# asharakeh/pod_compare

Measured on AMD Instinct MI355X. Metric: images/sec (BayesOD+MC-dropout, 1280x720), higher is better.
Workload: dtype f32 (convolutions: every fp32 product from 2-way f16 splits of the power-of-two-scaled fp32 operands, 3 partial products, fp32 accumulate; closer to fp64 than the fp32 MFMA: profiles/r05_f16_split_numerics.txt)

## Files before the change

pod_compare_amd/csrc/k12_wino_conv_split.hip:

```cpp
#include "pod_wino.h"

namespace pod {

typedef uint32_t vu32x4 __attribute__((ext_vector_type(4)));
constexpr int WINO_US_BYTES = 24 * 2 * 2 * 64 * 16;
constexpr int WINO_U_TOP = 14, WINO_V_TOP = 9;
constexpr int WINO_WAIT_VM24 = 0x4078;
constexpr int WINO_TAIL_NO_LOAD = 1, WINO_TAIL_NO_PARK = 2, WINO_TAIL_LAST = 4;

__global__ void __launch_bounds__(256) k_wino_filter_amax(const float* __restrict__ w, float* __restrict__ amax, int32_t K, int32_t C, int32_t Kpad) {
    const int64_t t = (int64_t)blockIdx.x * blockDim.x + threadIdx.x;
    float m = 0.0f;
    if (t < (int64_t)Kpad * C) {
        float u[4][6];
        wino_filter_values(w, (int)(t / C), (int)(t % C), K, C, u);
#pragma unroll
        for (int i = 0; i < 24; ++i) m = fmaxf(m, fabsf(u[i / 6][i % 6]));
    }
    wino_publish_amax1(amax, m);
}
__global__ void __launch_bounds__(256) k_wino_filter_split(const float* __restrict__ w, uint16_t* __restrict__ Us, const float* __restrict__ amax,
                                                           int32_t K, int32_t C, int32_t Kpad) {
    const int64_t t = (int64_t)blockIdx.x * blockDim.x + threadIdx.x;
    if (t >= (int64_t)Kpad * C) return;
    const int k = (int)(t / C), c = (int)(t % C);
    float u[4][6];
    wino_filter_values(w, k, c, K, C, u);
    const float sc = wino_pow2_scale(*amax, WINO_U_TOP);
    const int nchunk = C / 16, ks = k >> 6, kb = (k >> 5) & 1, j32 = k & 31, ch = c >> 4, hh = (c >> 3) & 1, e = c & 7;
    uint16_t* dst = Us + (((int64_t)ks * nchunk + ch) * (int64_t)WINO_US_BYTES) / 2 + (hh * 32 + j32) * 8 + e;
#pragma unroll
    for (int a = 0; a < 4; ++a)
#pragma unroll
        for (int p = 0; p < 6; ++p) {
            const float x = u[a][p] * sc;
            const _Float16 h0 = (_Float16)x;
            const _Float16 h1 = (_Float16)(x - (float)h0);
            uint16_t* d = dst + (((a * 6 + p) * 2 + kb) * 2) * 512;
            d[0] = __builtin_bit_cast(uint16_t, h0);
            d[512] = __builtin_bit_cast(uint16_t, h1);
        }
}

__global__ void __launch_bounds__(256, 1) k_wino_conv3x3_split(const WinoParams P) {
    extern __shared__ __attribute__((aligned(16))) float lds[];
    const int tid = threadIdx.x, lane = tid & 63, wave = tid >> 6;
    int ks, tb;
    wino_schedule(P.KS, P.n_blocks, ks, tb);
    if (tb >= P.n_blocks) return;
    uint32_t need[2] = {~0u, ~0u};
    if (P.live) {
        if (tb >= P.live[0]) return;
        const int32_t* const ent = P.live + POD_SPARSE_LIVE_HEAD + (int64_t)POD_SPARSE_LIVE_STRIDE * tb;
        tb = ent[0];
        need[0] = (uint32_t)ent[1 + (tid >> 5)];
        need[1] = (uint32_t)ent[9 + (tid >> 5 < 3 ? tid >> 5 : 2)];
    }
    WINO_STAMP(0);
    WINO_STAMP_WALL(12);
    uint32_t slot_e[12];
    int mini_pidx[3], dmini[3], doff[12];
    WINO_FILL_SLOTS(slot_e, mini_pidx, tid);
    const int nchunk_all = P.C >> 4;
    const int nchunk = P.c_split ? P.c_split : nchunk_all;
    const int chunk0 = (int)blockIdx.y * nchunk;
    const int i32 = lane & 31, h = lane >> 5;
    const int a = __builtin_amdgcn_readfirstlane(wave);
    const int set = (tb >= P.sets.first[1] ? 1 : 0) + (tb >= P.sets.first[2] ? 1 : 0) + (tb >= P.sets.first[3] ? 1 : 0);
    const float* const set_U = P.sets.U[set];
    const float* const set_in = P.sets.in[set];
    float* const set_out = P.sets.out[set];
    const float* const set_bias = P.sets.bias[set];
    const float in_amax_slot = wino_load_amax(P.sets.in_amax[set]);
    const float u_amax = *reinterpret_cast<const float*>(reinterpret_cast<const char*>(set_U) + (int64_t)P.KS * (P.C >> 4) * WINO_US_BYTES);
    float* const set_out_amax = P.sets.out_amax[set];
    const uint64_t set_offset = P.sets.offset[set];
    const int set_replicas = P.sets.replicas[set], set_k_planes = P.sets.k_planes[set];
    const auto u_rsrc = __builtin_amdgcn_make_buffer_rsrc(const_cast<char*>(reinterpret_cast<const char*>(set_U) + ((int64_t)ks * nchunk_all + chunk0) * WINO_US_BYTES), 0,
                                                          nchunk * WINO_US_BYTES, 0x00020000);
    const int u_off = (a * 6 * 4 * 64 + h * 32 + i32) * 16;
    constexpr int WINO_U_LEAD = 3;
    vu32x4 uP[6][4];
    auto filter_piece = [&](int q16, int p, vu32x4(&u)[4], int i) {
        u[i] = __builtin_bit_cast(vu32x4, __builtin_amdgcn_raw_buffer_load_b128(u_rsrc, u_off, q16 * WINO_US_BYTES + (p * 4 + i) * 1024, 0));
    };
#pragma unroll
    for (int pp = 0; pp < WINO_U_LEAD; ++pp)
#pragma unroll
        for (int i = 0; i < 4; ++i) filter_piece(0, pp, uP[pp], i);
    const WinoBlock B = wino_block(P.blocks[tb]);
    int row0, row1;
    float sgn;
    wino_rows(a, row0, row1, sgn);
    const int ty = i32 >> 2, tx = i32 & 3;
    const uint32_t lds_base = (uint32_t)(uintptr_t)(__attribute__((address_space(3))) float*)lds;
    uint32_t areg[2][2][2][2];
    uint32_t amini[2];
#pragma unroll
    for (int rs = 0; rs < 2; ++rs) {
        const int py = 2 * ty + (rs ? row1 : row0);
        const int p0 = 2 * (((py & 3) + 4 * (py >> 3)) * 18 + 4 * tx) + ((py >> 2) & 1);
#pragma unroll
        for (int cl = 0; cl < 2; ++cl) {
            const int rot = ((tx + cl) & 3) + 4 * ((py >> 1) & 1);
#pragma unroll
            for (int c16 = 0; c16 < 2; ++c16)
#pragma unroll
                for (int hf = 0; hf < 2; ++hf) areg[rs][cl][c16][hf] = lds_base + p0 * 128 + ((4 * c16 + 2 * h + hf + rot) & 7) * 16;
        }
    }
#pragma unroll
    for (int rs = 0; rs < 2; ++rs) amini[rs] = lds_base + 2 * WINO_SB_FLOATS * 4 + h * 12288 + ((2 * ty + (rs ? row1 : row0)) * 21 + tx) * 32;
    const auto r_rsrc = __builtin_amdgcn_make_buffer_rsrc(const_cast<float*>(set_in + B.base_px * P.in_stride + chunk0 * 16), 0,
                                                          B.n_img * B.HWi * P.in_stride * 4 - chunk0 * 64, 0x00020000);
    int* const pix_tab = wino_pixel_table(lds);
    WINO_FILL_PIXEL_TABLE(pix_tab, B, need, tid);
    wino_mini_offsets(&P, pix_tab, mini_pidx, dmini, lane);
    auto main_offsets = [&]() {
#pragma unroll
        for (int i = 0; i < 12; ++i) doff[i] = pix_tab[slot_e[i] & 0xFFFF];
#pragma unroll
        for (int i = 0; i < 12; ++i) doff[i] = wino_byte_offset(&P, doff[i], 4 * (((lane & 7) - (int)(slot_e[i] >> 16)) & 7));
    };

    f32x4 stg[6];
    const uint32_t stg_addr = lds_base + a * 12288 + lane * 16;
    auto stage_load = [&](int k, int sc, int i) {
        stg[k] = __builtin_bit_cast(f32x4, __builtin_amdgcn_raw_buffer_load_b128(r_rsrc, doff[i], sc * 128, 0));
    };
    auto stage_write = [&](int par, int k, int i) {
        *reinterpret_cast<__attribute__((address_space(3))) f32x4*>((uintptr_t)(stg_addr + par * (WINO_SB_FLOATS * 4) + i * 1024)) = stg[k];
    };

    f32x16 acc[12];
    f32x4 x[12];
    vu32x4 Vb[6][2];
    float tN[6][4], vN[2][6][4];
    if (POD_WINO_ELIM) {
#pragma unroll
    for (int i = 0; i < 12; ++i) Vb[i / 2][i % 2] = vu32x4{0x3c003c00u + i, 0x3c003c00u, 0x3c003c00u, 0x3c003c00u + lane};
#pragma unroll
    for (int i = 0; i < 12; ++i) x[i] = f32x4{1e-3f, 2e-3f, 3e-3f, 4e-3f} * (float)(lane + i);
#pragma unroll
    for (int i = 0; i < 48; ++i) vN[i / 24][(i / 4) % 6][i % 4] = x[i / 4][i % 4];
#pragma unroll
    for (int i = 0; i < 24; ++i) tN[i / 4][i % 4] = x[i / 4][i % 4];
    }
#define WINO_READ(par, c16, hf, i)                                                                                                  \
    asm volatile("ds_read_b128 %0, %1 offset:%2" : "=v"(x[i]) : "v"(areg[(i) / 6][((i) % 6) >> 2][c16][hf]), "i"((par) * WINO_SB_FLOATS * 4 + ((i) % 6) * 256))
#define WINO_READ_MINI(hf, i)                                                                                                        \
    asm volatile("ds_read_b128 %0, %1 offset:%2" : "=v"(x[i]) : "v"(amini[(i) / 6]), "i"((hf) * 16 + ((((i) % 6) & 3) * 5 + (((i) % 6) >> 2)) * 32))
#define WINO_READ12(M, ...)                                                                                                          \
    M(__VA_ARGS__, 0); M(__VA_ARGS__, 1); M(__VA_ARGS__, 2); M(__VA_ARGS__, 3); M(__VA_ARGS__, 4); M(__VA_ARGS__, 5);                \
    M(__VA_ARGS__, 6); M(__VA_ARGS__, 7); M(__VA_ARGS__, 8); M(__VA_ARGS__, 9); M(__VA_ARGS__, 10); M(__VA_ARGS__, 11)
#define WINO_READS_LANDED()                                                                                                           \
    asm volatile("s_waitcnt lgkmcnt(0)" : "+v"(x[0]), "+v"(x[1]), "+v"(x[2]), "+v"(x[3]), "+v"(x[4]), "+v"(x[5]), "+v"(x[6]), "+v"(x[7]), \
                 "+v"(x[8]), "+v"(x[9]), "+v"(x[10]), "+v"(x[11]))
    auto rows_combine = [&](int c0, int c1) __attribute__((always_inline)) {
#pragma unroll
        for (int c = c0; c < c1; ++c) {
#pragma unroll
            for (int e = 0; e < 4; ++e) tN[c][e] = __builtin_fmaf(sgn, x[6 + c][e], x[c][e]);
        }
    };
    float w0s[4], w1s[4], evs[4], ods[4], fs[4], gs[4];
    auto columns_level1 = [&](int e) __attribute__((always_inline)) {
        w0s[e] = __builtin_fmaf(-5.0f, tN[2][e], tN[4][e]);
        w1s[e] = __builtin_fmaf(-5.0f, tN[3][e], tN[5][e]);
        evs[e] = __builtin_fmaf(-4.0f, tN[2][e], tN[4][e]);
        ods[e] = __builtin_fmaf(-4.0f, tN[1][e], tN[3][e]);
        fs[e] = tN[4][e] - tN[2][e];
        gs[e] = tN[3][e] - tN[1][e];
    };
    auto columns_level2 = [&](int hf, int e) __attribute__((always_inline)) {
        vN[hf][0][e] = __builtin_fmaf(4.0f, tN[0][e], w0s[e]);
        vN[hf][5][e] = __builtin_fmaf(4.0f, tN[1][e], w1s[e]);
        vN[hf][1][e] = evs[e] + ods[e];
        vN[hf][2][e] = evs[e] - ods[e];
        vN[hf][3][e] = __builtin_fmaf(2.0f, gs[e], fs[e]);
        vN[hf][4][e] = __builtin_fmaf(-2.0f, gs[e], fs[e]);
    };
    const float sv = __builtin_bit_cast(float, __builtin_amdgcn_readfirstlane(__builtin_bit_cast(int, wino_pow2_scale(wino_reduce_amax(in_amax_slot), WINO_V_TOP))));
    auto split_convert = [&](int p, int term) __attribute__((always_inline)) {
        vu32x4 w;
#pragma unroll
        for (int i = 0; i < 4; ++i) {
            w[i] = term == 0 ? wino_f16_pair_scaled(vN[i >> 1][p][2 * (i & 1)], vN[i >> 1][p][2 * (i & 1) + 1], sv)
                             : wino_f16_pair(vN[i >> 1][p][2 * (i & 1)], vN[i >> 1][p][2 * (i & 1) + 1]);
        }
        Vb[p][term] = w;
    };
    auto split_residual = [&](int p, int i0, int i1) __attribute__((always_inline)) {
#pragma unroll
        for (int i = i0; i < i1; ++i) {
            float& lo = vN[i >> 1][p][2 * (i & 1)];
            float& hi = vN[i >> 1][p][2 * (i & 1) + 1];
            wino_f16_residual_scaled(Vb[p][0][i], lo, hi, sv);
        }
    };
    auto split_position = [&](int p) __attribute__((always_inline)) {
        split_convert(p, 0); split_residual(p, 0, 4); split_convert(p, 1);
    };
    auto make_v = [&](int hf) __attribute__((always_inline)) {
        if (POD_WINO_ELIM & 8) return;
        rows_combine(0, 6);
#pragma unroll
        for (int e = 0; e < 4; ++e) columns_level1(e);
#pragma unroll
        for (int e = 0; e < 4; ++e) columns_level2(hf, e);
    };
    auto split_all = [&]() __attribute__((always_inline)) {
        if (POD_WINO_ELIM & 8) return;
#pragma unroll
        for (int p = 0; p < 6; ++p) split_position(p);
    };

    constexpr int N_UNITS = 58, N_SLOTS = 36;
    auto unit = [&](auto U, auto npar_t, auto n16_t, auto hasA_t) __attribute__((always_inline)) {
        constexpr int u = decltype(U)::value, npar = decltype(npar_t)::value, n16 = decltype(n16_t)::value;
        if constexpr (POD_WINO_ELIM & 8) { if constexpr (u >= 3 && !(u >= 13 && u < 16)) return; }
        if constexpr (u < 3) {
            if constexpr (!(POD_WINO_ELIM & 1)) { WINO_READ(npar, n16, 0, 4 * u); WINO_READ(npar, n16, 0, 4 * u + 1); WINO_READ(npar, n16, 0, 4 * u + 2); WINO_READ(npar, n16, 0, 4 * u + 3); }
        } else if constexpr (u < 7) {
            if constexpr (decltype(hasA_t)::value) {
                constexpr int k = u - 3;
                if constexpr (k == 0) split_convert(5, 0);
                else if constexpr (k == 1) split_residual(5, 0, 2);
                else if constexpr (k == 2) split_residual(5, 2, 4);
                else split_convert(5, 1);
            }
        } else if constexpr (u < 13) {
            if constexpr (u == 7) WINO_READS_LANDED();
            rows_combine(u - 7, u - 6);
        } else if constexpr (u < 16) {
            if constexpr (!(POD_WINO_ELIM & 1)) { WINO_READ(npar, n16, 1, 4 * (u - 13)); WINO_READ(npar, n16, 1, 4 * (u - 13) + 1); WINO_READ(npar, n16, 1, 4 * (u - 13) + 2); WINO_READ(npar, n16, 1, 4 * (u - 13) + 3); }
        } else if constexpr (u < 24) {
            constexpr int k = u - 16;
            if constexpr (k < 4) columns_level1(k);
            else columns_level2(0, k - 4);
        } else if constexpr (u < 30) {
            if constexpr (u == 24) WINO_READS_LANDED();
            rows_combine(u - 24, u - 23);
        } else if constexpr (u < 38) {
            constexpr int k = u - 30;
            if constexpr (k < 4) columns_level1(k);
            else columns_level2(1, k - 4);
        } else {
            constexpr int p = (u - 38) / 4, k = (u - 38) % 4;
            if constexpr (k == 0) split_convert(p, 0);
            else if constexpr (k == 1) split_residual(p, 0, 2);
            else if constexpr (k == 2) split_residual(p, 2, 4);
            else split_convert(p, 1);
        }
    };
    const int last = nchunk - 1, last_s = last >> 1;
    const int sc1 = last_s < 1 ? last_s : 1;
#pragma unroll
    for (int r = 0; r < 3; ++r) wino_mini_piece(r_rsrc, lds, a, 0, r, dmini[r]);
#pragma unroll
    for (int r = 0; r < 3; ++r) wino_mini_piece(r_rsrc, lds, a, 1, r, dmini[r]);
    WINO_STAMP(9);
    main_offsets();
    WINO_STAMP(10);
#pragma unroll
    for (int i = 0; i < 12; ++i) wino_patch_piece(r_rsrc, lds, a, 0, i, doff[i]);
#pragma unroll
    for (int i = 0; i < 6; ++i) wino_patch_piece(r_rsrc, lds + WINO_SB_FLOATS, a, sc1, i, doff[i]);
#pragma unroll
    for (int i = 0; i < 6; ++i) stage_load(i, sc1, 6 + i);
    WINO_STAMP(11);
    __builtin_amdgcn_s_waitcnt(WINO_WAIT_VM24);
    __builtin_amdgcn_s_barrier();
    WINO_STAMP(1);
    WINO_READ12(WINO_READ_MINI, 0);
    WINO_READS_LANDED();
    __builtin_amdgcn_sched_barrier(0);
    make_v(0);
    __builtin_amdgcn_sched_barrier(0);
    WINO_READ12(WINO_READ_MINI, 1);
    WINO_READS_LANDED();
    __builtin_amdgcn_sched_barrier(0);
    make_v(1);
    split_all();
    __builtin_amdgcn_sched_barrier(0);
    WINO_STAMP(2);
    const f32x16 zero16 = {0.f, 0.f, 0.f, 0.f, 0.f, 0.f, 0.f, 0.f, 0.f, 0.f, 0.f, 0.f, 0.f, 0.f, 0.f, 0.f};
    auto chunk = [&](auto mode_t, auto c16_t, auto par_t, auto tail_t, int q) {
        constexpr int mode = decltype(mode_t)::value, c16 = decltype(c16_t)::value, par = decltype(par_t)::value, tail = decltype(tail_t)::value;
        constexpr bool do_load = !(tail & WINO_TAIL_NO_LOAD), do_park = !(tail & WINO_TAIL_NO_PARK), is_last = (tail & WINO_TAIL_LAST) != 0;
        static_assert((tail == 0 || mode == 2) && (!is_last || (!do_load && !do_park)), "tail forms are steady-state chunks; the last one has no stage traffic");
        constexpr int n16 = c16 ^ 1, npar = c16 == 1 ? par ^ 1 : par;
        const int qn = q + 1 <= last ? q + 1 : last;
        const int ls0 = (q >> 1) + 2, ls = ls0 < last_s ? ls0 : last_s;
        wino_static_for([&](auto J) __attribute__((always_inline)) {
            constexpr int j = decltype(J)::value, p = j / 6, m = j % 6, kb = m & 1, prod = m >> 1;
            constexpr int sa = prod == 1 ? 1 : 0;
            constexpr int sb = prod == 0 ? 1 : 0;
            if constexpr (mode == 0 && prod == 0)
                acc[p * 2 + kb] = __builtin_amdgcn_mfma_f32_32x32x16_f16(__builtin_bit_cast(wino_f16x8, uP[p][kb * 2 + sa]), __builtin_bit_cast(wino_f16x8, Vb[p][sb]), zero16, 0, 0, 0);
            else
                acc[p * 2 + kb] = __builtin_amdgcn_mfma_f32_32x32x16_f16(__builtin_bit_cast(wino_f16x8, uP[p][kb * 2 + sa]), __builtin_bit_cast(wino_f16x8, Vb[p][sb]), acc[p * 2 + kb], 0, 0, 0);
            if constexpr (m < 4 && (!is_last || p + WINO_U_LEAD < 6)) { if (!(POD_WINO_ELIM & 2)) filter_piece(p + WINO_U_LEAD >= 6 ? qn : q, (p + WINO_U_LEAD) % 6, uP[(p + WINO_U_LEAD) % 6], m); }
            if constexpr (m == 4 && do_park) { if (!(POD_WINO_ELIM & 4)) stage_write(c16 == 0 ? par ^ 1 : par, p, c16 == 0 ? 6 + p : p); }
            if constexpr (p == 5 && m >= 4 && do_load) {
                if (!(POD_WINO_ELIM & 4)) {
                    stage_load(3 * (m - 4), ls, 6 * c16 + 3 * (m - 4));
                    stage_load(3 * (m - 4) + 1, ls, 6 * c16 + 3 * (m - 4) + 1);
                    stage_load(3 * (m - 4) + 2, ls, 6 * c16 + 3 * (m - 4) + 2);
                }
            }
            if constexpr (mode != 0) {
                constexpr int u0 = j * N_UNITS / N_SLOTS, u1 = (j + 1) * N_UNITS / N_SLOTS;
                wino_static_for([&](auto K) __attribute__((always_inline)) {
                    constexpr int u = u0 + decltype(K)::value;
                    if constexpr (!is_last || (u >= 3 && u < 7))
                        unit(std::integral_constant<int, u>{}, std::integral_constant<int, npar>{}, std::integral_constant<int, n16>{}, std::integral_constant<bool, mode == 2>{});
                }, std::make_integer_sequence<int, u1 - u0>{});
            }
            __builtin_amdgcn_sched_barrier(0);
        }, std::make_integer_sequence<int, N_SLOTS>{});
        if constexpr (do_park) {
            __builtin_amdgcn_s_waitcnt(WINO_WAIT_LGKM0);
            __builtin_amdgcn_s_barrier();
        }
        if constexpr (mode == 0) {
            if (q >= last) return;
            if constexpr (!(POD_WINO_ELIM & 1)) WINO_READ12(WINO_READ, npar, n16, 0);
            WINO_READS_LANDED();
            __builtin_amdgcn_sched_barrier(0);
            make_v(0);
            __builtin_amdgcn_sched_barrier(0);
            if constexpr (!(POD_WINO_ELIM & 1)) WINO_READ12(WINO_READ, npar, n16, 1);
            WINO_READS_LANDED();
            __builtin_amdgcn_sched_barrier(0);
            make_v(1);
            split_all();
            __builtin_amdgcn_sched_barrier(0);
            __builtin_amdgcn_s_barrier();
        }
    };
    using std::integral_constant;
    constexpr integral_constant<int, 0> I0{};
    constexpr integral_constant<int, 1> I1{};
    constexpr integral_constant<int, 2> I2{};
    const bool peel = (nchunk & 3) == 0;
    const int nloop = peel ? nchunk - 4 : nchunk;
    chunk(I0, I0, I0, I0, 0);
    if (nchunk > 1) chunk(I1, I1, I0, I0, 1);
    for (int base = 0;; base += 4) {
#define WINO_CHUNK(t)                                                                                                              \
    if (base + (t) >= nloop) break;                                                                                                \
    chunk(I2, integral_constant<int, (t) & 1>{}, integral_constant<int, ((t) >> 1) & 1>{}, I0, base + (t));
        WINO_CHUNK(2) WINO_CHUNK(3) WINO_CHUNK(4) WINO_CHUNK(5)
#undef WINO_CHUNK
    }
    if (peel) {
        if (nchunk > 4) {
            chunk(I2, I0, I0, integral_constant<int, WINO_TAIL_NO_LOAD>{}, nchunk - 4);
            chunk(I2, I1, I0, integral_constant<int, WINO_TAIL_NO_LOAD | WINO_TAIL_NO_PARK>{}, nchunk - 3);
        }
        chunk(I2, I0, I1, integral_constant<int, WINO_TAIL_NO_LOAD | WINO_TAIL_NO_PARK>{}, nchunk - 2);
        chunk(I2, I1, I1, integral_constant<int, WINO_TAIL_NO_LOAD | WINO_TAIL_NO_PARK | WINO_TAIL_LAST>{}, nchunk - 1);
    }
    __syncthreads();
    WINO_STAMP(3);

    if (!wino_output_stage(acc, lds, a, i32, h)) return;
    const float inv = wino_pow2_inverse(sv) * wino_pow2_inverse(wino_pow2_scale(u_amax, WINO_U_TOP));
    const WinoStore S{set_out + (int64_t)blockIdx.y * P.split_out_stride, set_bias, set_out_amax, inv, set_offset, set_replicas, set_k_planes};
    const float lmax = S.k_planes > 0 ? wino_store_planes(P, B, S, lds, ks) : wino_store_channels_last(P, B, S, lds, ks);
    if (set_out_amax) wino_publish_amax_block(set_out_amax, lmax);
    WINO_STAMP_END();
}

}

#ifdef POD_TRACE
extern "C" int pod_wino_trace_dump_split(long long* host, int32_t n_workgroups) { return pod::wino_trace_dump(host, n_workgroups); }
#endif

extern "C" int64_t pod_wino_filter_split_bytes(int32_t K, int32_t C) {
    if (K < 1 || C < 16 || (C & 15) != 0) return 0;
    const int64_t Kpad = (K + 63) / 64 * 64;
    return Kpad / 64 * (C / 16) * (int64_t)pod::WINO_US_BYTES + 16;
}

extern "C" int pod_wino_filter_transform_split(const float* weight, void* Us, int32_t K, int32_t C, pod_stream_t stream) {
    if (!weight || !Us || K < 1 || C < 16 || (C & 15) != 0 || !pod_aligned(16, Us)) return POD_E_INVALID;
    const int32_t Kpad = (K + 63) / 64 * 64;
    const int64_t n = (int64_t)Kpad * C;
    float* amax = reinterpret_cast<float*>(reinterpret_cast<char*>(Us) + pod_wino_filter_split_bytes(K, C) - 16);
    if (hipMemsetAsync(amax, 0, 16, (hipStream_t)stream) != hipSuccess) return POD_E_LAUNCH;
    hipLaunchKernelGGL(pod::k_wino_filter_amax, dim3((unsigned)((n + 255) / 256)), dim3(256), 0, (hipStream_t)stream, weight, amax, K, C, Kpad);
    POD_CHECK_LAUNCH();
    hipLaunchKernelGGL(pod::k_wino_filter_split, dim3((unsigned)((n + 255) / 256)), dim3(256), 0, (hipStream_t)stream, weight,
                       reinterpret_cast<uint16_t*>(Us), amax, K, C, Kpad);
    POD_CHECK_LAUNCH();
    return POD_OK;
}

extern "C" int pod_wino_conv3x3_split(const PodWinoConv* d, pod_stream_t stream) {
    if (!d || d->n_sets < 1 || d->n_sets > 4 || !d->blocks || d->n_blocks < 0 || d->C < 16 || (d->C & 15) != 0 || d->K < 64 || (d->K & 63) != 0 ||
        !(d->p >= 0.0f && d->p < 1.0f) || d->sets[0].first_block != 0 || !pod_aligned(16, d->blocks) ||
        d->reserved != 0)
        return POD_E_INVALID;
    const int32_t C = d->C, K = d->K;
    pod::WinoParams P{};
    const int64_t grid = pod::wino_params_launch(P, d->blocks, d->n_blocks, C, K, d->relu, d->p, d->seed, d->epoch);
    if (grid < 0) return POD_E_INVALID;
    const bool partial = d->n_splits > 1;
    if (partial) {
        if (d->n_sets != 1 || d->n_splits > 16 || (C / 16) % d->n_splits != 0 || ((C / 16 / d->n_splits) & 1) != 0 || d->split_stride < 0 || (d->split_stride & 3) != 0 ||
            d->p != 0.0f || d->relu || d->sets[0].bias || d->sets[0].replicas || d->sets[0].k_planes || d->sets[0].out_amax)
            return POD_E_INVALID;
    }
    for (int s = 0; s < 4; ++s) {
        const PodConvSet& q = d->sets[s < d->n_sets ? s : 0];
        if (s < d->n_sets) {
            if (!q.in || !q.out || q.in == q.out || !q.Us || !q.in_amax || q.replicas < 0 || q.replicas > 127 || q.k_planes < 0 || q.k_planes > K ||
                (q.k_planes > 0 && (d->p != 0.0f || q.replicas != 0)) || (s > 0 && q.first_block < d->sets[s - 1].first_block) || q.first_block > d->n_blocks)
                return POD_E_INVALID;
            if (!pod_aligned(16, q.in, q.out, q.Us, q.bias) || !pod_aligned(4, q.in_amax, q.out_amax))
                return POD_E_INVALID;
        }
        pod::wino_params_set(P, s, s < d->n_sets ? q.first_block : INT32_MAX, q.in, q.out, q.Us, q.bias, q.in_amax, q.out_amax, q.offset, q.replicas, q.k_planes);
    }
    if (d->n_blocks == 0) return POD_OK;
    if (pod_lds_opt_in<pod::k_wino_conv3x3_split>(pod::WINO_LDS_BYTES) != POD_OK) return POD_E_LAUNCH;
    P.c_split = partial ? C / 16 / d->n_splits : 0; P.split_out_stride = partial ? d->split_stride : 0;
    P.live = d->live_blocks;
    hipLaunchKernelGGL(pod::k_wino_conv3x3_split, dim3((unsigned)grid, partial ? (unsigned)d->n_splits : 1u), dim3(256), pod::WINO_LDS_BYTES, (hipStream_t)stream, P);
    POD_CHECK_LAUNCH();
    return POD_OK;
}
```

pod_compare_amd/csrc/pod_wino.h:

```cpp
#pragma once
#include "pod_experiments.h"
#include "pod_split_gemm.h"

namespace pod {

constexpr int WINO_U_FLOATS = 24 * 2 * 64 * 4;
constexpr int WINO_SB_FLOATS = 384 * 32;
constexpr int WINO_LDS_BYTES = 4 * 32 * 4 * 65 * 4;

#ifdef POD_TRACE
static __device__ long long g_wino_trace[8192 * 16];
#define WINO_STAMP(k)                                                                                          \
    do {                                                                                                       \
        if (threadIdx.x == 0 && blockIdx.x < 8192) g_wino_trace[blockIdx.x * 16 + (k)] = __builtin_readcyclecounter(); \
    } while (0)
#define WINO_STAMP_WALL(k)                                                                                     \
    do {                                                                                                       \
        if (threadIdx.x == 0 && blockIdx.x < 8192) g_wino_trace[blockIdx.x * 16 + (k)] = wall_clock64();       \
    } while (0)
#define WINO_STAMP_END()                                                                                       \
    do {                                                                                                       \
        __builtin_amdgcn_s_waitcnt(0);                                                                         \
        WINO_STAMP(5);                                                                                         \
        WINO_STAMP_WALL(13);                                                                                   \
        if (threadIdx.x == 0 && blockIdx.x < 8192) {                                                           \
            uint32_t hw, xcc;                                                                                  \
            asm volatile("s_getreg_b32 %0, hwreg(HW_REG_HW_ID)" : "=s"(hw));                                   \
            asm volatile("s_getreg_b32 %0, hwreg(HW_REG_XCC_ID)" : "=s"(xcc));                                 \
            g_wino_trace[blockIdx.x * 16 + 6] = ((long long)xcc << 32) | hw;                                   \
        }                                                                                                      \
    } while (0)
static inline int wino_trace_dump(long long* host, int32_t n_workgroups) {
    if (hipDeviceSynchronize() != hipSuccess) return POD_E_LAUNCH;
    if (n_workgroups > 8192) n_workgroups = 8192;
    if (hipMemcpyFromSymbol(host, HIP_SYMBOL(g_wino_trace), (size_t)n_workgroups * 16 * sizeof(long long)) != hipSuccess) return POD_E_LAUNCH;
    return POD_OK;
}
#else
#define WINO_STAMP(k)
#define WINO_STAMP_WALL(k)
#define WINO_STAMP_END()
#endif

constexpr int WINO_WAIT_VM4 = 0x0074, WINO_WAIT_VM0 = 0x0070, WINO_WAIT_VM16 = 0x4070, WINO_WAIT_LGKM0 = 0xC07F;

struct WinoParams {
    const int4* blocks;
    int32_t n_blocks, C, K, KS, in_stride, out_stride, relu;
    uint32_t thresh;
    float scale;
    uint64_t seed;
    int32_t c_split;
    int64_t split_out_stride;
    const uint64_t* epoch;
    const int32_t* live;
    struct Sets {
        int32_t first[4];
        const float* in[4];
        float* out[4];
        const float* U[4];
        const float* bias[4];
        const float* in_amax[4];
        float* out_amax[4];
        uint64_t offset[4];
        int32_t replicas[4];
        int32_t k_planes[4];
    } sets;
};

struct WinoSlotTable {
    uint32_t v[384];
    constexpr WinoSlotTable() : v() {
        for (int p = 0; p < 384; ++p) {
            const int cls = p & 1, k = p >> 1, rr = k / 18, px = k - rr * 18;
            const int py = cls ? (rr < 4 ? rr + 4 : rr + 8) : (rr < 4 ? rr : rr < 8 ? rr + 4 : rr + 8);
            const bool ok = cls ? rr < 8 : rr < 10;
            v[p] = ok ? (uint32_t)((py * 18 + px) | ((((px >> 2) & 3) + 4 * ((py >> 1) & 1)) << 16)) : 324u;
        }
    }
};
static __device__ const WinoSlotTable g_wino_slots{};

__device__ __forceinline__ void wino_schedule(int KS, int n_blocks, int& ks, int& tb) {
    const int xcd = blockIdx.x & 7, wi = (int)(blockIdx.x >> 3);
    const int SP = KS >= 2 ? 2 : 1, G = KS / SP;
    ks = SP * (xcd % G) + (wi % SP);
    tb = (wi / SP) * (8 / G) + xcd / G;
}
inline int64_t wino_grid(int KS, int64_t n_blocks) {
    const int SP = KS >= 2 ? 2 : 1, G = KS / SP;
    return 8 * SP * ((n_blocks * G + 7) / 8);
}
inline int64_t wino_params_launch(WinoParams& P, const int32_t* blocks, int32_t n_blocks, int32_t C, int32_t K, int32_t relu, float p, uint64_t seed,
                                  const uint64_t* epoch) {
    const int32_t KS = K / 64;
    if (KS != 1 && KS != 2 && KS != 4 && KS != 8) return -1;
    P.blocks = reinterpret_cast<const int4*>(blocks);
    P.n_blocks = n_blocks; P.C = C; P.K = K; P.KS = KS; P.in_stride = C; P.out_stride = K; P.relu = relu;
    P.thresh = POD_DROPOUT_THRESH16(p);
    P.scale = 1.0f / (1.0f - p);
    P.seed = seed; P.epoch = epoch;
    const int64_t grid = wino_grid(KS, n_blocks);
    return grid > 0x7FFFFFFFLL ? -1 : grid;
}
inline void wino_params_set(WinoParams& P, int s, int32_t first, const float* in, float* out, const void* U, const float* bias, const float* in_amax,
                            float* out_amax, uint64_t offset, int32_t replicas, int32_t k_planes) {
    P.sets.first[s] = first;
    P.sets.in[s] = in; P.sets.out[s] = out; P.sets.U[s] = reinterpret_cast<const float*>(U); P.sets.bias[s] = bias;
    P.sets.in_amax[s] = in_amax; P.sets.out_amax[s] = out_amax;
    P.sets.offset[s] = offset; P.sets.replicas[s] = replicas; P.sets.k_planes[s] = k_planes;
}

template <typename T>
__device__ __forceinline__ void wino_pin_one(T& v) {
    asm volatile("" : "+v"(v));
}
template <typename... T>
__device__ __forceinline__ void wino_pin(T&... v) {
    (wino_pin_one(v), ...);
}

__device__ __forceinline__ void wino_filter_values(const float* __restrict__ w, int k, int c, int K, int C, float (&u)[4][6]) {
    float g[3][3];
#pragma unroll
    for (int i = 0; i < 9; ++i) g[i / 3][i % 3] = k < K ? w[((int64_t)k * C + c) * 9 + i] : 0.0f;
    float t0[4][3];
#pragma unroll
    for (int j = 0; j < 3; ++j) {
        t0[0][j] = g[0][j];
        t0[1][j] = 0.5f * (g[0][j] + g[1][j] + g[2][j]);
        t0[2][j] = 0.5f * (g[0][j] - g[1][j] + g[2][j]);
        t0[3][j] = g[2][j];
    }
#pragma unroll
    for (int a = 0; a < 4; ++a) {
        const float x0 = t0[a][0], x1 = t0[a][1], x2 = t0[a][2];
        u[a][0] = 0.25f * x0;
        u[a][1] = (-1.0f / 6.0f) * (x0 + x1 + x2);
        u[a][2] = (-1.0f / 6.0f) * (x0 - x1 + x2);
        u[a][3] = (1.0f / 24.0f) * x0 + (1.0f / 12.0f) * x1 + (1.0f / 6.0f) * x2;
        u[a][4] = (1.0f / 24.0f) * x0 - (1.0f / 12.0f) * x1 + (1.0f / 6.0f) * x2;
        u[a][5] = x2;
    }
}

struct WinoBlock {
    int64_t base_px, out_px;
    int gcols, H, W, n_img, y0, x0, Hv, Wv, HWi;
    float rHv, rWv;
};
__device__ __forceinline__ WinoBlock wino_block(const int4 desc) {
    WinoBlock B;
    B.base_px = desc.x; B.out_px = desc.y;
    B.gcols = (desc.z >> 24) & 0xFF; B.H = (desc.z >> 12) & 0xFFF; B.W = desc.z & 0xFFF; B.n_img = (desc.w >> 24) & 0xFF;
    B.y0 = ((desc.w >> 12) & 0xFFF) * 16; B.x0 = (desc.w & 0xFFF) * 16; B.Wv = B.W + 1; B.Hv = B.H + 1; B.HWi = B.H * B.W;
    B.rWv = 1.0f / (float)B.Wv; B.rHv = 1.0f / (float)B.Hv;
    return B;
}
__device__ __forceinline__ int wino_cell(int v, int step, float rstep, int& idx) {
    int n = (int)((float)v * rstep);
    n -= n * step > v ? 1 : 0;
    n += (n + 1) * step <= v ? 1 : 0;
    idx = n;
    return v - n * step;
}

__device__ __forceinline__ void wino_rows(int a, int& row0, int& row1, float& sgn) {
    row0 = a == 0 ? 0 : a == 2 ? 2 : 1;
    row1 = a == 2 ? 1 : a == 3 ? 3 : 2;
    sgn = a == 1 ? 1.0f : -1.0f;
}

__device__ __forceinline__ int* wino_pixel_table(float* lds) { return reinterpret_cast<int*>(lds + 2 * WINO_SB_FLOATS + 2 * 3072); }
#define WINO_FILL_PIXEL_TABLE(pix_tab, B, need, tid)                                                                                  \
    _Pragma("unroll") for (int it_ = 0; it_ < 2; ++it_) {                                                                             \
        const int t = (tid) + 256 * it_;                                                                                              \
        if (t >= 325) break;                                                                                                          \
        const int py = t / 18, px = t - py * 18, vy = (B).y0 - 1 + py, vx = (B).x0 - 1 + px;                                          \
        int m, n;                                                                                                                     \
        const int gy = wino_cell(vy < 0 ? 0 : vy, (B).Hv, (B).rHv, m), gx = wino_cell(vx < 0 ? 0 : vx, (B).Wv, (B).rWv, n), img = m * (B).gcols + n; \
        const bool ok = (t < 324) & (vy >= 0) & (gy < (B).H) & (vx >= 0) & (gx < (B).W) & (n < (B).gcols) & (img < (B).n_img) & ((((need)[it_] >> (t & 31)) & 1u) != 0); \
        (pix_tab)[t] = ok ? img * (B).HWi + gy * (B).W + gx : -1;       \
    }                                                                                                                                 \
    __syncthreads();                                                                                                                  \
    WINO_STAMP(8)

#define WINO_FILL_SLOTS(slot_e, mini_pidx, tid)                                                                                       \
    _Pragma("unroll") for (int i = 0; i < 12; ++i) (slot_e)[i] = g_wino_slots.v[96 * ((tid) >> 6) + 8 * i + (((tid) & 63) >> 3)];     \
    _Pragma("unroll") for (int r = 0; r < 3; ++r) {                                                                                   \
        const int pp = ((((tid) >> 6) * 3 + r) * 64 + ((tid) & 63)) >> 1, py = pp / 21, pi = pp - py * 21, px = 4 * (pi % 5) + pi / 5; \
        (mini_pidx)[r] = py < 18 && pi < 20 && px < 18 ? py * 18 + px : 324;                                                          \
    }
__device__ __forceinline__ int wino_byte_offset(const WinoParams* P, int pix, int part4) {
    return pix >= 0 ? (pix * P->in_stride + part4) * 4 : 0x7FFFFF00;
}
__device__ __forceinline__ void wino_mini_offsets(const WinoParams* P, const int* pix_tab, const int (&mini_pidx)[3], int (&dmini)[3], int lane) {
#pragma unroll
    for (int r = 0; r < 3; ++r) dmini[r] = pix_tab[mini_pidx[r]];
#pragma unroll
    for (int r = 0; r < 3; ++r) dmini[r] = wino_byte_offset(P, dmini[r], 4 * (lane & 1));
}
typedef __attribute__((address_space(3))) void wino_lds_void;
__device__ __forceinline__ void wino_mini_piece(__amdgpu_buffer_rsrc_t rsrc, float* lds, int a, int which, int r, int dmini_r) {
    __builtin_amdgcn_raw_ptr_buffer_load_lds(rsrc, (wino_lds_void*)(lds + 2 * WINO_SB_FLOATS + which * 3072 + (a * 3 + r) * 256), 16, dmini_r, which * 32, 0, 0);
}
__device__ __forceinline__ void wino_patch_piece(__amdgpu_buffer_rsrc_t rsrc, float* stage, int a, int sc, int i, int doff_i) {
    __builtin_amdgcn_raw_ptr_buffer_load_lds(rsrc, (wino_lds_void*)(stage + (a * 12 + i) * 256), 16, doff_i, sc * 128, 0, 0);
}

constexpr int WINO_TS = 260;
constexpr int WINO_ZA = 32 * WINO_TS;
__device__ __forceinline__ bool wino_output_stage(const f32x16 (&acc)[12], float* lds, int a, int i32, int h) {
    if (POD_WINO_ELIM & 128) {
#pragma unroll
        for (int i = 0; i < 12; ++i) asm volatile("" ::"v"(acc[i]));
        return false;
    }
#pragma unroll
    for (int kb = 0; kb < 2; ++kb)
#pragma unroll
        for (int g = 0; g < 4; ++g) {
            f32x4 m[6];
#pragma unroll
            for (int p6 = 0; p6 < 6; ++p6) m[p6] = f32x4{acc[p6 * 2 + kb][4 * g], acc[p6 * 2 + kb][4 * g + 1], acc[p6 * 2 + kb][4 * g + 2], acc[p6 * 2 + kb][4 * g + 3]};
            const f32x4 s1 = m[1] + m[2], d1 = m[1] - m[2], s2 = m[3] + m[4], d2 = m[3] - m[4];
            float* o = lds + (a * 32 + i32) * WINO_TS + kb * 32 + 8 * g + 4 * h;
            *reinterpret_cast<f32x4*>(o) = (m[0] + s1) + s2;
            *reinterpret_cast<f32x4*>(o + 64) = __builtin_elementwise_fma(f32x4{2.f, 2.f, 2.f, 2.f}, d2, d1);
            *reinterpret_cast<f32x4*>(o + 128) = __builtin_elementwise_fma(f32x4{4.f, 4.f, 4.f, 4.f}, s2, s1);
            *reinterpret_cast<f32x4*>(o + 192) = __builtin_elementwise_fma(f32x4{8.f, 8.f, 8.f, 8.f}, d2, d1) + m[5];
        }
    __syncthreads();
    WINO_STAMP(4);
    return !(POD_WINO_ELIM & 32);
}

struct WinoStore {
    float* out;
    const float* bias;
    float* out_amax;
    float inv;
    uint64_t offset;
    int replicas, k_planes;
};
__device__ __forceinline__ void wino_dropout8(f32x4& v0, f32x4& v1, int64_t e, uint64_t offset, uint32_t word, uint64_t key, uint32_t thresh, float scale) {
    const uint64_t ctr = offset + (uint64_t)(e >> 3);
    const u32x4 r4 = philox4x32_10(u32x4{(uint32_t)ctr, (uint32_t)(ctr >> 32), word, STREAM_DROPOUT}, (uint32_t)key, (uint32_t)(key >> 32));
    dropout_mask4(v0, r4.x, r4.y, thresh, scale);
    dropout_mask4(v1, r4.z, r4.w, thresh, scale);
}


template <bool RELU, bool AMAX>
__device__ __forceinline__ float wino_store_planes_form(const WinoBlock& B, const WinoStore& S, const float* lds, int ks) {
    const int tid = threadIdx.x, wave = __builtin_amdgcn_readfirstlane(tid >> 6);
    float lmax = 0.0f;
    const f32x4 inv = f32x4{S.inv, S.inv, S.inv, S.inv};
    const int oy = (tid >> 2) & 15, ox = (tid & 3) * 4, odd = oy & 1;
    const float sg = odd ? -1.0f : 1.0f;
    const int kg0 = ks * 64 + wave;
    const int n_it = (S.k_planes - kg0 + 3) >> 2;
    const float bias_l = S.bias ? S.bias[kg0 + 4 * (tid & 15)] : 0.0f;
    int m;
    const int gy = wino_cell(B.y0 + oy, B.Hv, B.rHv, m);
    int64_t px0[4];
#pragma unroll
    for (int e = 0; e < 4; ++e) {
        int n;
        const int gx = wino_cell(B.x0 + ox + e, B.Wv, B.rWv, n), img = m * B.gcols + n;
        px0[e] = (n < B.gcols && img < B.n_img && gx < B.W && gy < B.H) ? (B.out_px + (int64_t)img * B.HWi) * S.k_planes + (int64_t)gy * B.W + gx : -1;
    }
    const bool vec = px0[0] >= 0 && px0[3] == px0[0] + 3 && (px0[0] & 3) == 0 && (B.HWi & 3) == 0;
    const bool ok[4] = {px0[0] >= 0, px0[1] >= 0, px0[2] >= 0, px0[3] >= 0};
    int64_t q[4];
#pragma unroll
    for (int e = 0; e < 4; ++e) q[e] = (int64_t)kg0 * B.HWi + px0[e];
    const int64_t q_it = (int64_t)4 * B.HWi;
    const int tile = (oy >> 1) * 4 + (tid & 3);
    const float* r = lds + tile * WINO_TS + wave + (odd ? WINO_ZA : 0);
#pragma unroll 1
    for (int it0 = 0; it0 < 16 && it0 < n_it; it0 += 4, r += 16) {
        float z[4][4][3];
        f32x4 v[4];
#pragma unroll
        for (int j = 0; j < 4; ++j)
#pragma unroll
            for (int e = 0; e < 4; ++e)
#pragma unroll
                for (int a = 0; a < 3; ++a) z[j][e][a] = r[4 * j + e * 64 + a * WINO_ZA];
#pragma unroll
        for (int j = 0; j < 4; ++j) {
            const float bias = __builtin_bit_cast(float, __builtin_amdgcn_readlane(__builtin_bit_cast(int, bias_l), it0 + j));
            f32x4 y;
#pragma unroll
            for (int e = 0; e < 4; ++e) y[e] = __builtin_fmaf(sg, z[j][e][2], __builtin_fmaf(sg, z[j][e][1], z[j][e][0]));
            v[j] = __builtin_elementwise_fma(y, inv, f32x4{bias, bias, bias, bias});
            if (RELU) wino_relu4(v[j]);
            if (AMAX) {
                const float mx = wino_absmax4(0.0f, f32x4{ok[0] ? v[j].x : 0.f, ok[1] ? v[j].y : 0.f, ok[2] ? v[j].z : 0.f, ok[3] ? v[j].w : 0.f});
                lmax = fmaxf(lmax, it0 + j < n_it ? mx : 0.0f);
            }
        }
        wino_pin(v[0], v[1], v[2], v[3]);
#pragma unroll
        for (int j = 0; j < 4; ++j) {
            const bool live = it0 + j < n_it;
            if (live && vec) {
                *reinterpret_cast<f32x4*>(S.out + q[0]) = v[j];
            } else if (live) {
                if (ok[0]) S.out[q[0]] = v[j].x;
                if (ok[1]) S.out[q[1]] = v[j].y;
                if (ok[2]) S.out[q[2]] = v[j].z;
                if (ok[3]) S.out[q[3]] = v[j].w;
            }
#pragma unroll
            for (int e = 0; e < 4; ++e) q[e] += q_it;
        }
    }
    return lmax;
}
__device__ __forceinline__ float wino_store_planes(const WinoParams& P, const WinoBlock& B, const WinoStore& S, const float* lds, int ks) {
    switch ((P.relu ? 1 : 0) | (S.out_amax ? 2 : 0)) {
        case 0: return wino_store_planes_form<false, false>(B, S, lds, ks);
        case 1: return wino_store_planes_form<true, false>(B, S, lds, ks);
        case 2: return wino_store_planes_form<false, true>(B, S, lds, ks);
        default: return wino_store_planes_form<true, true>(B, S, lds, ks);
    }
}

template <bool RELU, bool DROP>
__device__ __forceinline__ float wino_store_channels_last_form(const WinoParams& P, const WinoBlock& B, const WinoStore& S, const float* lds, int ks) {
    const int tid = threadIdx.x;
    float lmax = 0.0f;
    const f32x4 inv = f32x4{S.inv, S.inv, S.inv, S.inv};
    const int k8 = (tid & 7) * 8, kg = ks * 64 + k8, ox = (tid >> 3) & 15, odd = tid >> 7;
    const float sg1 = odd ? -1.0f : 1.0f;
    const f32x4 sg = f32x4{sg1, sg1, sg1, sg1};
    f32x4 bias0 = f32x4{0.f, 0.f, 0.f, 0.f}, bias1 = bias0;
    if (S.bias) {
        bias0 = *reinterpret_cast<const f32x4*>(S.bias + kg);
        bias1 = *reinterpret_cast<const f32x4*>(S.bias + kg + 4);
    }
    const uint64_t drop_key = DROP ? dropout_key(P.seed, P.epoch) : 0ull;
    const int n_rep = S.replicas > 0 ? S.replicas : 1;
    const uint32_t word = S.replicas > 0 ? 2u : 0u;
    int n, m;
    const int gx = wino_cell(B.x0 + ox, B.Wv, B.rWv, n);
    const bool col_ok = n < B.gcols && gx < B.W;
    int gy = wino_cell(B.y0 + odd, B.Hv, B.rHv, m);
    int img = m * B.gcols + n;
    const int64_t e_row = (int64_t)(2 * B.W) * P.out_stride, e_wrap = ((int64_t)B.gcols * B.HWi - (int64_t)B.Hv * B.W) * P.out_stride, e_rep = (int64_t)B.HWi * P.out_stride;
    int64_t e = (B.out_px + (int64_t)img * B.HWi + (int64_t)gy * B.W + gx) * P.out_stride + kg - e_row;
    gy -= 2;
    const float* rbase = lds + (ox >> 2) * WINO_TS + (ox & 3) * 64 + k8 + (odd ? WINO_ZA : 0);
#pragma unroll 1
    for (int g = 0; g < 2; ++g) {
        f32x4 z[4][6], v[4][2];
        bool ok[4];
        int64_t er[4];
#pragma unroll
        for (int it = 0; it < 4; ++it) {
            gy += 2;
            const bool wrap = gy >= B.Hv;
            gy -= wrap ? B.Hv : 0;
            img += wrap ? B.gcols : 0;
            e += e_row + (wrap ? e_wrap : 0);
            ok[it] = col_ok && gy < B.H && img < B.n_img;
            er[it] = e;
            const float* r = rbase + (4 * g + it) * 4 * WINO_TS;
            z[it][0] = *reinterpret_cast<const f32x4*>(r); z[it][1] = *reinterpret_cast<const f32x4*>(r + 4);
            z[it][2] = *reinterpret_cast<const f32x4*>(r + WINO_ZA); z[it][3] = *reinterpret_cast<const f32x4*>(r + WINO_ZA + 4);
            z[it][4] = *reinterpret_cast<const f32x4*>(r + 2 * WINO_ZA); z[it][5] = *reinterpret_cast<const f32x4*>(r + 2 * WINO_ZA + 4);
        }
#pragma unroll
        for (int it = 0; it < 4; ++it) {
            v[it][0] = __builtin_elementwise_fma(__builtin_elementwise_fma(sg, z[it][4], __builtin_elementwise_fma(sg, z[it][2], z[it][0])), inv, bias0);
            v[it][1] = __builtin_elementwise_fma(__builtin_elementwise_fma(sg, z[it][5], __builtin_elementwise_fma(sg, z[it][3], z[it][1])), inv, bias1);
            if (RELU) {
                wino_relu4(v[it][0]);
                wino_relu4(v[it][1]);
            }
            const float mx = wino_absmax4(wino_absmax4(0.0f, v[it][0]), v[it][1]);
            lmax = fmaxf(lmax, ok[it] ? (DROP ? mx * P.scale : mx) : 0.0f);
        }
#pragma unroll 1
        for (int rep = 0; rep < n_rep; ++rep) {
            f32x4 w[4][2];
#pragma unroll
            for (int it = 0; it < 4; ++it) {
                w[it][0] = v[it][0];
                w[it][1] = v[it][1];
                if (DROP && !(POD_WINO_ELIM & 64)) wino_dropout8(w[it][0], w[it][1], er[it], S.offset, word, drop_key, P.thresh, P.scale);
            }
#pragma unroll
            for (int it = 0; it < 4; ++it) wino_pin(w[it][0], w[it][1]);
#pragma unroll
            for (int it = 0; it < 4; ++it) {
                if (ok[it]) {
                    *reinterpret_cast<f32x4*>(S.out + er[it]) = w[it][0];
                    *reinterpret_cast<f32x4*>(S.out + er[it] + 4) = w[it][1];
                }
                er[it] += e_rep;
            }
        }
    }
    return lmax;
}
__device__ __forceinline__ float wino_store_channels_last(const WinoParams& P, const WinoBlock& B, const WinoStore& S, const float* lds, int ks) {
    switch ((P.relu ? 1 : 0) | (P.thresh ? 2 : 0)) {
        case 0: return wino_store_channels_last_form<false, false>(P, B, S, lds, ks);
        case 1: return wino_store_channels_last_form<true, false>(P, B, S, lds, ks);
        case 2: return wino_store_channels_last_form<false, true>(P, B, S, lds, ks);
        default: return wino_store_channels_last_form<true, true>(P, B, S, lds, ks);
    }
}

}
```

Baseline: 144.3.

## Drop mini-patch prologue and start Winograd pipeline directly from staged chunk

```diff
diff --git a/pod_compare_amd/csrc/k12_wino_conv_split.hip b/pod_compare_amd/csrc/k12_wino_conv_split.hip
--- a/pod_compare_amd/csrc/k12_wino_conv_split.hip
+++ b/pod_compare_amd/csrc/k12_wino_conv_split.hip
@@ -5,7 +5,7 @@
 typedef uint32_t vu32x4 __attribute__((ext_vector_type(4)));
 constexpr int WINO_US_BYTES = 24 * 2 * 2 * 64 * 16;
 constexpr int WINO_U_TOP = 14, WINO_V_TOP = 9;
-constexpr int WINO_WAIT_VM24 = 0x4078;
+constexpr int WINO_WAIT_VM12 = 0x007C;
 constexpr int WINO_TAIL_NO_LOAD = 1, WINO_TAIL_NO_PARK = 2, WINO_TAIL_LAST = 4;
 
 __global__ void __launch_bounds__(256) k_wino_filter_amax(const float* __restrict__ w, float* __restrict__ amax, int32_t K, int32_t C, int32_t Kpad) {
@@ -59,7 +59,7 @@
     WINO_STAMP(0);
     WINO_STAMP_WALL(12);
     uint32_t slot_e[12];
-    int mini_pidx[3], dmini[3], doff[12];
+    int mini_pidx[3], doff[12];
     WINO_FILL_SLOTS(slot_e, mini_pidx, tid);
     const int nchunk_all = P.C >> 4;
     const int nchunk = P.c_split ? P.c_split : nchunk_all;
@@ -95,7 +95,6 @@
     const int ty = i32 >> 2, tx = i32 & 3;
     const uint32_t lds_base = (uint32_t)(uintptr_t)(__attribute__((address_space(3))) float*)lds;
     uint32_t areg[2][2][2][2];
-    uint32_t amini[2];
 #pragma unroll
     for (int rs = 0; rs < 2; ++rs) {
         const int py = 2 * ty + (rs ? row1 : row0);
@@ -109,18 +108,15 @@
                 for (int hf = 0; hf < 2; ++hf) areg[rs][cl][c16][hf] = lds_base + p0 * 128 + ((4 * c16 + 2 * h + hf + rot) & 7) * 16;
         }
     }
-#pragma unroll
-    for (int rs = 0; rs < 2; ++rs) amini[rs] = lds_base + 2 * WINO_SB_FLOATS * 4 + h * 12288 + ((2 * ty + (rs ? row1 : row0)) * 21 + tx) * 32;
     const auto r_rsrc = __builtin_amdgcn_make_buffer_rsrc(const_cast<float*>(set_in + B.base_px * P.in_stride + chunk0 * 16), 0,
                                                           B.n_img * B.HWi * P.in_stride * 4 - chunk0 * 64, 0x00020000);
     int* const pix_tab = wino_pixel_table(lds);
-    WINO_FILL_PIXEL_TABLE(pix_tab, B, need, tid);
-    wino_mini_offsets(&P, pix_tab, mini_pidx, dmini, lane);
+    WINO_FILL_PIXEL_TABLE_BYTES(pix_tab, B, need, tid, P.in_stride);
     auto main_offsets = [&]() {
 #pragma unroll
         for (int i = 0; i < 12; ++i) doff[i] = pix_tab[slot_e[i] & 0xFFFF];
 #pragma unroll
-        for (int i = 0; i < 12; ++i) doff[i] = wino_byte_offset(&P, doff[i], 4 * (((lane & 7) - (int)(slot_e[i] >> 16)) & 7));
+        for (int i = 0; i < 12; ++i) doff[i] += 16 * (((lane & 7) - (int)(slot_e[i] >> 16)) & 7);
     };
 
     f32x4 stg[6];
@@ -148,8 +144,6 @@
     }
 #define WINO_READ(par, c16, hf, i)                                                                                                  \
     asm volatile("ds_read_b128 %0, %1 offset:%2" : "=v"(x[i]) : "v"(areg[(i) / 6][((i) % 6) >> 2][c16][hf]), "i"((par) * WINO_SB_FLOATS * 4 + ((i) % 6) * 256))
-#define WINO_READ_MINI(hf, i)                                                                                                        \
-    asm volatile("ds_read_b128 %0, %1 offset:%2" : "=v"(x[i]) : "v"(amini[(i) / 6]), "i"((hf) * 16 + ((((i) % 6) & 3) * 5 + (((i) % 6) >> 2)) * 32))
 #define WINO_READ12(M, ...)                                                                                                          \
     M(__VA_ARGS__, 0); M(__VA_ARGS__, 1); M(__VA_ARGS__, 2); M(__VA_ARGS__, 3); M(__VA_ARGS__, 4); M(__VA_ARGS__, 5);                \
     M(__VA_ARGS__, 6); M(__VA_ARGS__, 7); M(__VA_ARGS__, 8); M(__VA_ARGS__, 9); M(__VA_ARGS__, 10); M(__VA_ARGS__, 11)
@@ -255,10 +249,6 @@
     };
     const int last = nchunk - 1, last_s = last >> 1;
     const int sc1 = last_s < 1 ? last_s : 1;
-#pragma unroll
-    for (int r = 0; r < 3; ++r) wino_mini_piece(r_rsrc, lds, a, 0, r, dmini[r]);
-#pragma unroll
-    for (int r = 0; r < 3; ++r) wino_mini_piece(r_rsrc, lds, a, 1, r, dmini[r]);
     WINO_STAMP(9);
     main_offsets();
     WINO_STAMP(10);
@@ -269,15 +259,15 @@
 #pragma unroll
     for (int i = 0; i < 6; ++i) stage_load(i, sc1, 6 + i);
     WINO_STAMP(11);
-    __builtin_amdgcn_s_waitcnt(WINO_WAIT_VM24);
+    __builtin_amdgcn_s_waitcnt(WINO_WAIT_VM12);
     __builtin_amdgcn_s_barrier();
     WINO_STAMP(1);
-    WINO_READ12(WINO_READ_MINI, 0);
+    WINO_READ12(WINO_READ, 0, 0, 0);
     WINO_READS_LANDED();
     __builtin_amdgcn_sched_barrier(0);
     make_v(0);
     __builtin_amdgcn_sched_barrier(0);
-    WINO_READ12(WINO_READ_MINI, 1);
+    WINO_READ12(WINO_READ, 0, 0, 1);
     WINO_READS_LANDED();
     __builtin_amdgcn_sched_barrier(0);
     make_v(1);
@@ -288,7 +278,7 @@
     auto chunk = [&](auto mode_t, auto c16_t, auto par_t, auto tail_t, int q) {
         constexpr int mode = decltype(mode_t)::value, c16 = decltype(c16_t)::value, par = decltype(par_t)::value, tail = decltype(tail_t)::value;
         constexpr bool do_load = !(tail & WINO_TAIL_NO_LOAD), do_park = !(tail & WINO_TAIL_NO_PARK), is_last = (tail & WINO_TAIL_LAST) != 0;
-        static_assert((tail == 0 || mode == 2) && (!is_last || (!do_load && !do_park)), "tail forms are steady-state chunks; the last one has no stage traffic");
+        static_assert((tail == 0 || mode == 1) && (!is_last || (!do_load && !do_park)), "tail forms are steady-state chunks; the last one has no stage traffic");
         constexpr int n16 = c16 ^ 1, npar = c16 == 1 ? par ^ 1 : par;
         const int qn = q + 1 <= last ? q + 1 : last;
         const int ls0 = (q >> 1) + 2, ls = ls0 < last_s ? ls0 : last_s;
@@ -309,12 +299,12 @@
                     stage_load(3 * (m - 4) + 2, ls, 6 * c16 + 3 * (m - 4) + 2);
                 }
             }
-            if constexpr (mode != 0) {
+            {
                 constexpr int u0 = j * N_UNITS / N_SLOTS, u1 = (j + 1) * N_UNITS / N_SLOTS;
                 wino_static_for([&](auto K) __attribute__((always_inline)) {
                     constexpr int u = u0 + decltype(K)::value;
                     if constexpr (!is_last || (u >= 3 && u < 7))
-                        unit(std::integral_constant<int, u>{}, std::integral_constant<int, npar>{}, std::integral_constant<int, n16>{}, std::integral_constant<bool, mode == 2>{});
+                        unit(std::integral_constant<int, u>{}, std::integral_constant<int, npar>{}, std::integral_constant<int, n16>{}, std::integral_constant<bool, mode != 0>{});
                 }, std::make_integer_sequence<int, u1 - u0>{});
             }
             __builtin_amdgcn_sched_barrier(0);
@@ -323,44 +313,27 @@
             __builtin_amdgcn_s_waitcnt(WINO_WAIT_LGKM0);
             __builtin_amdgcn_s_barrier();
         }
-        if constexpr (mode == 0) {
-            if (q >= last) return;
-            if constexpr (!(POD_WINO_ELIM & 1)) WINO_READ12(WINO_READ, npar, n16, 0);
-            WINO_READS_LANDED();
-            __builtin_amdgcn_sched_barrier(0);
-            make_v(0);
-            __builtin_amdgcn_sched_barrier(0);
-            if constexpr (!(POD_WINO_ELIM & 1)) WINO_READ12(WINO_READ, npar, n16, 1);
-            WINO_READS_LANDED();
-            __builtin_amdgcn_sched_barrier(0);
-            make_v(1);
-            split_all();
-            __builtin_amdgcn_sched_barrier(0);
-            __builtin_amdgcn_s_barrier();
-        }
     };
     using std::integral_constant;
     constexpr integral_constant<int, 0> I0{};
     constexpr integral_constant<int, 1> I1{};
-    constexpr integral_constant<int, 2> I2{};
     const bool peel = (nchunk & 3) == 0;
-    const int nloop = peel ? nchunk - 4 : nchunk;
+    const int nloop = peel ? (nchunk > 4 ? nchunk - 4 : 2) : nchunk;
     chunk(I0, I0, I0, I0, 0);
-    if (nchunk > 1) chunk(I1, I1, I0, I0, 1);
     for (int base = 0;; base += 4) {
 #define WINO_CHUNK(t)                                                                                                              \
     if (base + (t) >= nloop) break;                                                                                                \
-    chunk(I2, integral_constant<int, (t) & 1>{}, integral_constant<int, ((t) >> 1) & 1>{}, I0, base + (t));
-        WINO_CHUNK(2) WINO_CHUNK(3) WINO_CHUNK(4) WINO_CHUNK(5)
+    chunk(I1, integral_constant<int, (t) & 1>{}, integral_constant<int, ((t) >> 1) & 1>{}, I0, base + (t));
+        WINO_CHUNK(1) WINO_CHUNK(2) WINO_CHUNK(3) WINO_CHUNK(4)
 #undef WINO_CHUNK
     }
     if (peel) {
         if (nchunk > 4) {
-            chunk(I2, I0, I0, integral_constant<int, WINO_TAIL_NO_LOAD>{}, nchunk - 4);
-            chunk(I2, I1, I0, integral_constant<int, WINO_TAIL_NO_LOAD | WINO_TAIL_NO_PARK>{}, nchunk - 3);
-        }
-        chunk(I2, I0, I1, integral_constant<int, WINO_TAIL_NO_LOAD | WINO_TAIL_NO_PARK>{}, nchunk - 2);
-        chunk(I2, I1, I1, integral_constant<int, WINO_TAIL_NO_LOAD | WINO_TAIL_NO_PARK | WINO_TAIL_LAST>{}, nchunk - 1);
+            chunk(I1, I0, I0, integral_constant<int, WINO_TAIL_NO_LOAD>{}, nchunk - 4);
+            chunk(I1, I1, I0, integral_constant<int, WINO_TAIL_NO_LOAD | WINO_TAIL_NO_PARK>{}, nchunk - 3);
+        }
+        chunk(I1, I0, I1, integral_constant<int, WINO_TAIL_NO_LOAD | WINO_TAIL_NO_PARK>{}, nchunk - 2);
+        chunk(I1, I1, I1, integral_constant<int, WINO_TAIL_NO_LOAD | WINO_TAIL_NO_PARK | WINO_TAIL_LAST>{}, nchunk - 1);
     }
     __syncthreads();
     WINO_STAMP(3);
diff --git a/pod_compare_amd/csrc/pod_wino.h b/pod_compare_amd/csrc/pod_wino.h
--- a/pod_compare_amd/csrc/pod_wino.h
+++ b/pod_compare_amd/csrc/pod_wino.h
@@ -172,7 +172,10 @@
 }
 
 __device__ __forceinline__ int* wino_pixel_table(float* lds) { return reinterpret_cast<int*>(lds + 2 * WINO_SB_FLOATS + 2 * 3072); }
-#define WINO_FILL_PIXEL_TABLE(pix_tab, B, need, tid)                                                                                  \
+constexpr int WINO_NO_PIXEL = 0x7FFFFF00;
+#define WINO_FILL_PIXEL_TABLE(pix_tab, B, need, tid) WINO_FILL_PIXEL_TABLE_AS(pix_tab, B, need, tid, , -1)
+#define WINO_FILL_PIXEL_TABLE_BYTES(pix_tab, B, need, tid, in_stride) WINO_FILL_PIXEL_TABLE_AS(pix_tab, B, need, tid, * (in_stride) * 4, WINO_NO_PIXEL)
+#define WINO_FILL_PIXEL_TABLE_AS(pix_tab, B, need, tid, SCALED, NONE)                                                                 \
     _Pragma("unroll") for (int it_ = 0; it_ < 2; ++it_) {                                                                             \
         const int t = (tid) + 256 * it_;                                                                                              \
         if (t >= 325) break;                                                                                                          \
@@ -180,7 +183,7 @@
         int m, n;                                                                                                                     \
         const int gy = wino_cell(vy < 0 ? 0 : vy, (B).Hv, (B).rHv, m), gx = wino_cell(vx < 0 ? 0 : vx, (B).Wv, (B).rWv, n), img = m * (B).gcols + n; \
         const bool ok = (t < 324) & (vy >= 0) & (gy < (B).H) & (vx >= 0) & (gx < (B).W) & (n < (B).gcols) & (img < (B).n_img) & ((((need)[it_] >> (t & 31)) & 1u) != 0); \
-        (pix_tab)[t] = ok ? img * (B).HWi + gy * (B).W + gx : -1;       \
+        (pix_tab)[t] = ok ? (img * (B).HWi + gy * (B).W + gx) SCALED : NONE;       \
     }                                                                                                                                 \
     __syncthreads();                                                                                                                  \
     WINO_STAMP(8)
@@ -192,7 +195,7 @@
         (mini_pidx)[r] = py < 18 && pi < 20 && px < 18 ? py * 18 + px : 324;                                                          \
     }
 __device__ __forceinline__ int wino_byte_offset(const WinoParams* P, int pix, int part4) {
-    return pix >= 0 ? (pix * P->in_stride + part4) * 4 : 0x7FFFFF00;
+    return pix >= 0 ? (pix * P->in_stride + part4) * 4 : WINO_NO_PIXEL;
 }
 __device__ __forceinline__ void wino_mini_offsets(const WinoParams* P, const int* pix_tab, const int (&mini_pidx)[3], int (&dmini)[3], int lane) {
 #pragma unroll
```

Result: no change. 143.9, median of 3 (-0.3%).
